# Deltares/pyflwdir

Measured on AMD Instinct MI355X. Metric: Mcells/s upstream_area on D8 raster, higher is better.
Workload: dtype int32

## Files before the change

pyflwdir_amd/csrc/tile_fast.h:

```cpp
#pragma once
#include <type_traits>

#define FX_SLOT0 (2u * TCELLS)
#define FX_NOBODY (FX_SLOT0 + 2u * PSL)
#define FX_PN (TCELLS + PSL + 8)
#ifndef FXP
#define FXP 4
#endif
#define FY_SINK0 (4u * TCELLS)

#define FX_TP_LO 0x3F404101u
#define FX_TP_HI 0xC1C0BFFFu
#define FX_TC_LO 0x47484901u
#define FX_TC_HI 0xB9B8B7FFu
#define FX_T0_LO 0xF7F70000u
#define FX_T0_HI 0xF7F7F7F7u

__device__ __forceinline__ u32 fx_ffbl(u32 x) {
  u32 r;
  asm("v_ffbl_b32 %0, %1" : "=v"(r) : "v"(x));
  return r;
}
__device__ __forceinline__ int fx_sext8(u32 x) { return (int)(int8_t)(x & 0xFFu); }

__device__ __forceinline__ u32 fx_rowmask(u32 lr) { return (lr == 0u ? 0xE0u : 0u) | (lr == TS - 1u ? 0x0Eu : 0u); }
__device__ __forceinline__ u32 fx_colmask(u32 lc) { return (lc == 0u ? 0x38u : 0u) | (lc == TS - 1u ? 0x83u : 0u); }

__device__ __forceinline__ bool fx_vote(u32 (*s_flag)[4], int round, u32 tid, bool live) {
  const bool any = __ballot(live) != 0ull;
  if ((tid & 63u) == 0u) s_flag[round & 1][tid >> 6] = any ? 1u : 0u;
  __syncthreads();
  const uint4 f = *(const uint4 *)s_flag[round & 1];
  return (f.x | f.y | f.z | f.w) != 0u;
}

struct NbrTab {
  uint16_t v[PSL][8];
};
constexpr NbrTab make_nbr_tab() {
  NbrTab t{};
  for (int p = 0; p < PSL; ++p) {
    int lr = 0, lc = 0;
    if (p < TS) lr = 0, lc = p;
    else if (p < 2 * TS) lr = TS - 1, lc = p - TS;
    else if (p < 2 * TS + (TS - 2)) lr = p - 2 * TS + 1, lc = 0;
    else lr = p - (2 * TS + (TS - 2)) + 1, lc = TS - 1;
    int cnt = 0;
    for (int k = 0; k < 8 && p < NPERIM; ++k) {
      const int dr = (k >= 1 && k <= 3) ? 1 : (k >= 5 ? -1 : 0);
      const int dc = (k == 0 || k == 1 || k == 7) ? 1 : ((k >= 3 && k <= 5) ? -1 : 0);
      const int nr = lr + dr, nc = lc + dc;
      if (nr >= 0 && nr < TS && nc >= 0 && nc < TS) continue;
      const int qr = nr & (TS - 1), qc = nc & (TS - 1);
      const int ps = qr == 0 ? qc : (qr == TS - 1 ? TS + qc : (qc == 0 ? 2 * TS + (qr - 1) : 2 * TS + (TS - 2) + (qr - 1)));
      const int d = 3 * ((nr < 0 ? -1 : (nr >= TS ? 1 : 0)) + 1) + (nc < 0 ? -1 : (nc >= TS ? 1 : 0)) + 1;
      t.v[p][cnt++] = (uint16_t)(ps | (d << 8) | (k << 12));
    }
    for (; cnt < 8; ++cnt) t.v[p][cnt] = (uint16_t)((p < NPERIM ? p : 0) | (4 << 8) | (8 << 12));
  }
  return t;
}
static __device__ __constant__ const NbrTab NBR_TAB = make_nbr_tab();

__device__ __forceinline__ u64 w_cell(u64 base, u32 f, u32 c) { return base + (u64)(__umulhi(c + 1u, f) - __umulhi(c, f)); }


template <int NW>
__device__ __forceinline__ bool fx_vote_n(u32 (*s_flag)[8], int round, u32 tid, bool live) {
  const bool any = __ballot(live) != 0ull;
  if ((tid & 63u) == 0u) s_flag[round & 1][tid >> 6] = any ? 1u : 0u;
  __syncthreads();
  const uint4 f = *(const uint4 *)s_flag[round & 1];
  u32 acc = f.x | f.y | f.z | f.w;
  if (NW == 8) {
    const uint4 g = *(const uint4 *)&s_flag[round & 1][4];
    acc |= g.x | g.y | g.z | g.w;
  }
  return acc != 0u;
}

template <bool RAW, bool WEIGHTS, bool WIDE = false>
__global__ void __launch_bounds__(256) k_tile_local_fast(TileArgs a) {
  __shared__ __attribute__((aligned(16))) u32 A[PSL * FXP];
  __shared__ __attribute__((aligned(16))) u64 A64[WIDE ? PSL * 4 : 2];
  __shared__ __attribute__((aligned(16))) uint16_t P[FX_PN];
  __shared__ __attribute__((aligned(16))) u8 code[HW * CP];
  __shared__ __attribute__((aligned(16))) u32 s_flag[2][4];
  __shared__ u64 s_cnt[4];
  const u32 tid = threadIdx.x;
  u32 bx_, by_;
  pfd_tile_of_block(&bx_, &by_);
  const u32 tc = bx_ + a.tc_lo, tr = by_ + a.tr_lo;
  const u32 sbase = sslot_base(tr, tc, a.nstc);
  const i64 r0 = (i64)tr * TS, c0 = (i64)tc * TS;
  bool mvq = false;
  {
    u32 v[5];
    stage_load_interior(RAW ? a.raw : a.ncode, a.ncol, r0, c0, tid, v);
    if (RAW) {
#pragma unroll
      for (int k = 0; k < 5; ++k) {
        const u32 x = v[k] ^ 0xF7F7F7F7u;
        mvq |= ((x - 0x01010101u) & ~x & 0x80808080u) != 0u;
      }
    }
    stage_store(code, tid, v);
  }
  *(uint4 *)&A[FXP * tid] = make_uint4(0u, 0u, 0u, 0u);
  if (FXP == 8) *(uint4 *)&A[FXP * tid + 4] = make_uint4(0u, 0u, 0u, 0u);
  if (WIDE) {
#pragma unroll
    for (int k = 0; k < 4; ++k) A64[tid + 256u * k] = 0;
  }
  P[TCELLS + tid] = (uint16_t)(FX_SLOT0 + 2u * tid);
  if (tid == 0) P[TCELLS + PSL] = (uint16_t)FX_NOBODY;
  const bool tile_mv = RAW ? (__syncthreads_or(mvq ? 1 : 0) != 0) : (__syncthreads(), false);

  const u32 qs = (tid >> 3) & 3u;
  const u32 lcq = 4u * (tid & 15u);
  u32 sh[4], cm[4];
#pragma unroll
  for (int s = 0; s < 4; ++s) {
    const u32 b = (u32)s ^ qs;
    sh[s] = 8u * b;
    cm[s] = fx_colmask(lcq + b);
  }
  u32 ndir = 0, npit = 0, nbad = 0;
  auto decode = [&](auto chk) {
  constexpr bool CHKMV = decltype(chk)::value;
#pragma unroll
  for (int j = 0; j < QPT; ++j) {
    const u32 lr = (tid >> 4) + 16u * j;
    const u32 l0 = 4u * tid + 1024u * j;
    const u32 ca0 = (lr + 1u) * CP + lcq + 4u;
    const u32 c4 = *(const u32 *)&code[ca0];
    const u32 rm = (j == 0 || j == QPT - 1) ? fx_rowmask(lr) : 0u;
    u32 p[4], n4 = 0, badq = 0;
#pragma unroll
    for (int s = 0; s < 4; ++s) {
      const u32 c = (c4 >> sh[s]) & 0xFFu;
      const u32 k = fx_ffbl(c);
      const u32 pcnt = __popc(c);
      bool isdir = pcnt == 1u;
      if (RAW) {
        if (CHKMV) {
          const u32 t = code[(u32)((int)(ca0 + (sh[s] >> 3)) + fx_sext8(__builtin_amdgcn_perm(FX_TC_HI, FX_TC_LO, k)))];
          isdir = isdir && t != D8_MV;
        }
        const u32 t0 = __builtin_amdgcn_perm(FX_T0_HI, FX_T0_LO, pcnt);
        const u32 n = isdir ? c : t0;
        badq |= t0 & ~c;
        n4 |= n << sh[s];
        ndir += isdir ? 1u : 0u;
        npit += n == 0u ? 1u : 0u;
      }
      const bool go = isdir && (c & (rm | cm[s])) == 0u;
      const u32 lt = (u32)((int)(l0 + (sh[s] >> 3)) + fx_sext8(__builtin_amdgcn_perm(FX_TP_HI, FX_TP_LO, k)));
      p[s] = go ? (PHYS(lt) << 1) : FX_NOBODY;
    }
    *(uint2 *)&P[l0] = make_uint2(p[0] | (p[1] << 16), p[2] | (p[3] << 16));
    if (RAW) {
      if (badq) {
#pragma unroll
        for (int s = 0; s < 4; ++s) {
          const u32 c = (c4 >> sh[s]) & 0xFFu;
          nbad += (__builtin_amdgcn_perm(FX_T0_HI, FX_T0_LO, __popc(c)) & ~c) ? 1u : 0u;
        }
      }
      *(u32 *)&code[ca0] = n4;
      __builtin_memcpy(a.ncode_w + (size_t)(r0 + lr) * a.ncol + (size_t)(c0 + lcq), &n4, 4);
    }
  }
  };
  if (RAW && tile_mv) decode(std::true_type{});
  else decode(std::false_type{});
  if (RAW) {
    u64 pk = (u64)(ndir + npit) | ((u64)npit << 16) | ((u64)nbad << 32);
    for (int o = 32; o > 0; o >>= 1) pk += __shfl_down(pk, o);
    if ((tid & 63u) == 0) s_cnt[tid >> 6] = pk;
  }
  __syncthreads();
  if (RAW && tid == 0) a.tcnt[(size_t)tr * a.ntc + tc] = s_cnt[0] + s_cnt[1] + s_cnt[2] + s_cnt[3];

  u32 xt12 = XR_NONE;
  int plr = 0, plc = 0;
  if (tid < NPERIM) {
    pslot_inv((int)tid, &plr, &plc);
    const u32 c = CODE(plr, plc);
    if (d8_is_dir(c)) {
      const int k = d8_slot(c);
      const int nr = plr + d8_dr(k), nc = plc + d8_dc(k);
      if ((unsigned)nr >= TS || (unsigned)nc >= TS) {
        xt12 = xr_t12(nr, nc);
        P[PHYS((u32)(plr * TS + plc))] = (uint16_t)(FX_SLOT0 + 2u * tid);
      }
    }
  }
  __syncthreads();

  u32 pc[QPT * 4];
  bool lv[QPT];
#pragma unroll
  for (int j = 0; j < QPT; ++j) {
    const uint2 pp = *(const uint2 *)&P[4u * tid + 1024u * j];
    pc[4 * j + 0] = pp.x & 0xFFFFu;
    pc[4 * j + 1] = pp.x >> 16;
    pc[4 * j + 2] = pp.y & 0xFFFFu;
    pc[4 * j + 3] = pp.y >> 16;
    lv[j] = !(pp.x & pp.y & (pp.x >> 16) & (pp.y >> 16) & FX_SLOT0);
  }
  int round = 0;
#pragma nounroll
  for (; round < MAXROUNDS_TILE; ++round) {
#pragma unroll
    for (int j = 0; j < QPT; ++j) {
      if (lv[j]) {
        u32 q[4];
#pragma unroll
        for (int b = 0; b < 4; ++b) q[b] = *(const uint16_t *)((const u8 *)P + pc[4 * j + b]);
#pragma unroll
        for (int b = 0; b < 4; ++b) q[b] = *(const uint16_t *)((const u8 *)P + q[b]);
#pragma unroll
        for (int b = 0; b < 4; ++b) pc[4 * j + b] = q[b];
        lv[j] = !(q[0] & q[1] & q[2] & q[3] & FX_SLOT0);
        *(uint2 *)&P[4u * tid + 1024u * j] = make_uint2(q[0] | (q[1] << 16), q[2] | (q[3] << 16));
      }
    }
    if (!fx_vote(s_flag, round, tid, lv[0] | lv[1] | lv[2] | lv[3])) break;
  }
  const u32 live = (lv[0] ? 1u : 0u) + (lv[1] ? 1u : 0u) + (lv[2] ? 1u : 0u) + (lv[3] ? 1u : 0u);
  if ((a.flags & 32) && tid == 0) {
    const unsigned long long r = (unsigned long long)min(round + 1, MAXROUNDS_TILE);
    const u32 w = (tr * a.ntc + tc) & 255u;
    atomicMax((unsigned long long *)&a.rcnt[w], r);
    atomicAdd((unsigned long long *)&a.rcnt[256 + w], r);
  }
  if (live) atomicAdd((unsigned long long *)&a.ctrl[T_UNSAT], (unsigned long long)live);

  const u32 rep = 4u * (tid & (FXP - 1u));
#pragma unroll
  for (int j = 0; j < QPT; ++j) {
    u32 x[4], w[4];
#pragma unroll
    for (int s = 0; s < 4; ++s) {
      x[s] = pc[4 * j + s] - FX_SLOT0;
      w[s] = x[s] < 2u * PSL ? 1u : 0u;
      if (WEIGHTS) {
        const u32 lr = (tid >> 4) + 16u * j;
        w[s] = x[s] < 2u * PSL ? (u32)a.weights[(size_t)(r0 + lr) * a.ncol + (size_t)(c0 + lcq + (sh[s] >> 3))] : 0u;
      }
    }
    const bool e10 = x[1] == x[0], e20 = x[2] == x[0], e21 = x[2] == x[1], e30 = x[3] == x[0], e31 = x[3] == x[1], e32 = x[3] == x[2];
    w[0] += (e10 ? w[1] : 0u) + (e20 ? w[2] : 0u) + (e30 ? w[3] : 0u);
    w[1] = e10 ? 0u : w[1] + ((!e20 && e21) ? w[2] : 0u) + ((!e30 && e31) ? w[3] : 0u);
    w[2] = (e20 || e21) ? 0u : w[2] + ((!e30 && !e31 && e32) ? w[3] : 0u);
    w[3] = (e30 || e31 || e32) ? 0u : w[3];
#pragma unroll
    for (int s = 0; s < 4; ++s)
      if (w[s]) atomicAdd((u32 *)((u8 *)A + (x[s] << (FXP == 8 ? 4 : 3)) + rep), w[s]);
    if (WIDE) {
      const u32 lr = (tid >> 4) + 16u * j;
      const u64 wr = a.wrow[(u32)(r0 + lr)];
      const u32 wf = a.wfrac[(u32)(r0 + lr)];
      u64 v[4];
#pragma unroll
      for (int s = 0; s < 4; ++s) v[s] = x[s] < 2u * PSL ? w_cell(wr, wf, (u32)c0 + lcq + (sh[s] >> 3)) : 0ull;
      const bool e10 = x[1] == x[0], e20 = x[2] == x[0], e21 = x[2] == x[1], e30 = x[3] == x[0], e31 = x[3] == x[1], e32 = x[3] == x[2];
      v[0] += (e10 ? v[1] : 0ull) + (e20 ? v[2] : 0ull) + (e30 ? v[3] : 0ull);
      v[1] = e10 ? 0ull : v[1] + ((!e20 && e21) ? v[2] : 0ull) + ((!e30 && e31) ? v[3] : 0ull);
      v[2] = (e20 || e21) ? 0ull : v[2] + ((!e30 && !e31 && e32) ? v[3] : 0ull);
      v[3] = (e30 || e31 || e32) ? 0ull : v[3];
#pragma unroll
      for (int s = 0; s < 4; ++s)
        if (v[s]) atomicAdd((unsigned long long *)&A64[(x[s] >> 1) * 4u + (tid & 3u)], (unsigned long long)v[s]);
    }
  }
  __syncthreads();

  u32 xt = 0, link = XR_NONE, inmask = 0;
  if (tid < NPERIM) {
    if (xt12 != XR_NONE) {
      const uint4 lo = *(const uint4 *)&A[tid * FXP];
      xt = lo.x + lo.y + lo.z + lo.w;
      if (FXP == 8) {
        const uint4 hi = *(const uint4 *)&A[tid * FXP + 4];
        xt += hi.x + hi.y + hi.z + hi.w;
      }
    }
    const u32 c = CODE(plr, plc);
    if (c != D8_MV) {
#pragma unroll
      for (int k = 0; k < 8; ++k) {
        const int nr = plr + d8_dr(k), nc = plc + d8_dc(k);
        if (((unsigned)nr >= TS || (unsigned)nc >= TS) && CODE(nr, nc) == (1u << ((k + 4) & 7))) inmask |= 1u << k;
      }
    }
    if (inmask) {
      const u32 x = (u32)P[PHYS((u32)(plr * TS + plc))] - FX_SLOT0;
      if (x < 2u * PSL) link = x >> 1;
    }
  }
  a.xT[sbase + tid] = xt;
  a.xrec[sbase + tid] = xr_pack(xt12 & 0xFFu, xt12 >> 8, link, inmask);
  if (WIDE) a.xT64[sbase + tid] = (tid < NPERIM && xt12 != XR_NONE) ? A64[4u * tid] + A64[4u * tid + 1] + A64[4u * tid + 2] + A64[4u * tid + 3] : 0ull;
  const u64 xm = __ballot(xt12 != XR_NONE);
  if ((tid & 63u) == 0u) a.xmask[(sbase + tid) >> 6] = xm;
}

template <bool WEIGHTS, int NT>
__global__ void __launch_bounds__(NT, NT == 256 ? 6 : 8) k_tile_final_fast(TileArgs a) {
  constexpr int QF = TCELLS / 4 / NT;
  constexpr u32 QSTR = 4u * NT;
  constexpr u32 RSTR = NT / 16;
  constexpr int NW = NT / 64;
  __shared__ __attribute__((aligned(16))) u32 A[TCELLS + 64];
  __shared__ __attribute__((aligned(16))) uint16_t P[TCELLS + 64];
  __shared__ __attribute__((aligned(16))) u32 s_flag[2][8];
  const u32 tid = threadIdx.x;
  u32 bx_, by_;
  pfd_tile_of_block(&bx_, &by_);
  const u32 tc = bx_ + a.tc_lo, tr = by_ + a.tr_lo;
  const u32 sbase = sslot_base(tr, tc, a.nstc);
  const i64 r0 = (i64)tr * TS, c0 = (i64)tc * TS;
  const u32 lcq = 4u * (tid & 15u);
  u32 cq[QF];
#pragma unroll
  for (int j = 0; j < QF; ++j)
    __builtin_memcpy(&cq[j], a.ncode + (size_t)(r0 + (tid >> 4) + RSTR * j) * a.ncol + (size_t)(c0 + lcq), 4);
  const u32 ptid = tid & 255u;
  const u32 rec = tid < 256u ? a.xrec[sbase + ptid] : 0u;
  u32 xc[5], xk[5];
  {
    const uint4 nb = *reinterpret_cast<const uint4 *>(NBR_TAB.v[ptid]);
    const u32 dl = min(tid & 15u, 8u), ql = (dl * 11u) >> 5;
    const u32 nbase = sslot_base(tr + ql - 1u, tc + (dl - 3u * ql) - 1u, a.nstc);
    const u32 e5[5] = {nb.x & 0xFFFFu, nb.x >> 16, nb.y & 0xFFFFu, nb.y >> 16, nb.z & 0xFFFFu};
#pragma unroll
    for (int i = 0; i < 5; ++i) {
      const u32 bs = (u32)__shfl((int)nbase, (int)(((tid & 48u) | ((e5[i] >> 8) & 15u))));
      xc[i] = a.xtot[bs + (e5[i] & 0xFFu)];
      xk[i] = e5[i] >> 12;
    }
  }
  const u32 sink = FY_SINK0 + 4u * (tid & 63u);
  if (tid < 64u) P[TCELLS + tid] = (uint16_t)sink;

  const u32 qs = (tid >> 3) & 3u;
  u32 sh[4], cm[4];
#pragma unroll
  for (int s = 0; s < 4; ++s) {
    const u32 b = (u32)s ^ qs;
    sh[s] = 8u * b;
    cm[s] = fx_colmask(lcq + b);
  }
  u32 pc[QF * 4], qn[QF * 4];
  bool lv[QF];
#pragma unroll
  for (int j = 0; j < QF; ++j) {
    const u32 lr = (tid >> 4) + RSTR * j;
    const u32 l0 = 4u * tid + QSTR * j;
    const u32 c4 = cq[j];
    const u32 rm = (j == 0 || j == QF - 1) ? fx_rowmask(lr) : 0u;
    u32 w4[4];
#pragma unroll
    for (int s = 0; s < 4; ++s) {
      const u32 c = (c4 >> sh[s]) & 0xFFu;
      const bool go = __popc(c & ~(rm | cm[s])) == 1u;
      const u32 lt = (u32)((int)(l0 + (sh[s] >> 3)) + fx_sext8(__builtin_amdgcn_perm(FX_TP_HI, FX_TP_LO, fx_ffbl(c))));
      pc[4 * j + s] = go ? (PHYS(lt) << 2) : sink;
      u32 wv = 1u;
      if (WEIGHTS) wv = (u32)a.weights[(size_t)(r0 + lr) * a.ncol + (size_t)(c0 + lcq + (sh[s] >> 3))];
      w4[s] = c != D8_MV ? wv : 0u;
    }
    *(uint4 *)&A[l0] = make_uint4(w4[0], w4[1], w4[2], w4[3]);
    *(uint2 *)&P[l0] = make_uint2(pc[4 * j + 0] | (pc[4 * j + 1] << 16), pc[4 * j + 2] | (pc[4 * j + 3] << 16));
    lv[j] = !(pc[4 * j + 0] & pc[4 * j + 1] & pc[4 * j + 2] & pc[4 * j + 3] & FY_SINK0);
  }
  u32 inf = 0;
  {
    const u32 m = (rec >> 16) & 0xFFu;
#pragma unroll
    for (int i = 0; i < 5; ++i) inf += ((m >> xk[i]) & 1u) ? xc[i] : 0u;
  }
  __syncthreads();
  if (inf) {
    int plr, plc;
    pslot_inv((int)ptid, &plr, &plc);
    A[PHYS((u32)(plr * TS + plc))] += inf;
  }
  __syncthreads();

#define FY_ROUND(PC, QN)                                                                                                \
  {                                                                                                               \
    u32 av[QF * 4];                                                                                              \
    _Pragma("unroll") for (int j = 0; j < QF; ++j) {                                                              \
      if (lv[j]) {                                                                                                \
        const uint4 a4 = *(const uint4 *)&A[4u * tid + QSTR * j];                                                  \
        av[4 * j + 0] = a4.x, av[4 * j + 1] = a4.y, av[4 * j + 2] = a4.z, av[4 * j + 3] = a4.w;                   \
        _Pragma("unroll") for (int b = 0; b < 4; ++b)                                                             \
            QN[4 * j + b] = *(const uint16_t *)((const u8 *)P + (PC[4 * j + b] >> 1));                           \
      }                                                                                                           \
    }                                                                                                             \
    __syncthreads();                            \
    _Pragma("unroll") for (int j = 0; j < QF; ++j) {                                                              \
      if (lv[j]) {                                                                                                \
         \
         \
        const u32 t0 = PC[4 * j], t1 = PC[4 * j + 1], t2 = PC[4 * j + 2], t3 = PC[4 * j + 3];                     \
        u32 w0 = av[4 * j], w1 = av[4 * j + 1], w2 = av[4 * j + 2], w3 = av[4 * j + 3];                           \
        const bool e10 = t1 == t0, e20 = t2 == t0, e21 = t2 == t1, e30 = t3 == t0, e31 = t3 == t1, e32 = t3 == t2; \
        w0 += (e10 ? w1 : 0u) + (e20 ? w2 : 0u) + (e30 ? w3 : 0u);                                                \
        w1 = e10 ? 0u : w1 + ((!e20 && e21) ? w2 : 0u) + ((!e30 && e31) ? w3 : 0u);                               \
        w2 = (e20 || e21) ? 0u : w2 + ((!e30 && !e31 && e32) ? w3 : 0u);                                          \
        w3 = (e30 || e31 || e32) ? 0u : w3;                                                                       \
        atomicAdd((u32 *)((u8 *)A + t0), w0);                                                                     \
        if (w1) atomicAdd((u32 *)((u8 *)A + t1), w1);                                                             \
        if (w2) atomicAdd((u32 *)((u8 *)A + t2), w2);                                                             \
        if (w3) atomicAdd((u32 *)((u8 *)A + t3), w3);                                                             \
        lv[j] = !(QN[4 * j + 0] & QN[4 * j + 1] & QN[4 * j + 2] & QN[4 * j + 3] & FY_SINK0);                      \
        *(uint2 *)&P[4u * tid + QSTR * j] =                                                                       \
            make_uint2(QN[4 * j + 0] | (QN[4 * j + 1] << 16), QN[4 * j + 2] | (QN[4 * j + 3] << 16));             \
      }                                                                                                           \
    }                                                                                                             \
  }
  auto anylive = [&]() {
    bool v = false;
    _Pragma("unroll") for (int j = 0; j < QF; ++j) v |= lv[j];
    return v;
  };
  int round = 0;
#pragma nounroll
  for (; round < MAXROUNDS_TILE; round += 2) {
    FY_ROUND(pc, qn)
    if (!fx_vote_n<NW>(s_flag, 0, tid, anylive())) break;
    FY_ROUND(qn, pc)
    if (!fx_vote_n<NW>(s_flag, 1, tid, anylive())) {
      ++round;
      break;
    }
  }
#undef FY_ROUND
  u32 live = 0;
  _Pragma("unroll") for (int j = 0; j < QF; ++j) live += lv[j] ? 1u : 0u;
  if ((a.flags & 32) && tid == 0) {
    const unsigned long long r = (unsigned long long)min(round + 1, MAXROUNDS_TILE);
    const u32 w = (tr * a.ntc + tc) & 255u;
    atomicMax((unsigned long long *)&a.rcnt[512 + w], r);
    atomicAdd((unsigned long long *)&a.rcnt[768 + w], r);
  }
  if (live) atomicAdd((unsigned long long *)&a.ctrl[T_UNSAT], (unsigned long long)live);

#pragma unroll
  for (int j = 0; j < QF; ++j) {
    const u32 l0 = 4u * tid + QSTR * j;
    const u32 c4 = cq[j];
    const uint4 a4 = *(const uint4 *)&A[l0];
    const u32 x0 = (qs & 1u) ? a4.y : a4.x, x1 = (qs & 1u) ? a4.x : a4.y;
    const u32 x2 = (qs & 1u) ? a4.w : a4.z, x3 = (qs & 1u) ? a4.z : a4.w;
    i32 o4[4] = {(i32)((qs & 2u) ? x2 : x0), (i32)((qs & 2u) ? x3 : x1), (i32)((qs & 2u) ? x0 : x2),
                 (i32)((qs & 2u) ? x1 : x3)};
#pragma unroll
    for (int b = 0; b < 4; ++b)
      if (((c4 >> (8 * b)) & 0xFFu) == D8_MV) o4[b] = -9999;
    i32 *dst = a.out + (size_t)(r0 + (tid >> 4) + RSTR * j - a.row_first) * a.ncol + (size_t)(c0 + lcq);
    if ((((size_t)dst) & 15) == 0) {
      *(int4 *)dst = make_int4(o4[0], o4[1], o4[2], o4[3]);
    } else {
#pragma unroll
      for (int b = 0; b < 4; ++b) dst[b] = o4[b];
    }
  }
}
```

Baseline: 214,800.

## Use ds_write_addtid stores and split even/odd planes for tile pointer array

```diff
diff --git a/pyflwdir_amd/csrc/tile_fast.h b/pyflwdir_amd/csrc/tile_fast.h
--- a/pyflwdir_amd/csrc/tile_fast.h
+++ b/pyflwdir_amd/csrc/tile_fast.h
@@ -79,6 +79,25 @@
   return acc != 0u;
 }
 
+__device__ __forceinline__ u32 fx_lds_addr(const void *p) {
+  return (u32)(__UINTPTR_TYPE__)(__attribute__((address_space(3))) const void *)p;
+}
+#pragma clang diagnostic push
+#pragma clang diagnostic ignored "-Winline-asm"
+__device__ __forceinline__ void fx_st_addtid(u32 m0, u32 d) {
+  asm volatile("s_mov_b32 m0, %1\n\ts_nop 0\n\tds_write_addtid_b32 %0" : : "v"(d), "s"(m0) : "m0", "memory");
+}
+__device__ __forceinline__ void fx_st2_addtid(u32 m0, u32 d0, u32 d1) {
+  asm volatile("s_mov_b32 m0, %2\n\ts_nop 0\n\tds_write_addtid_b32 %0\n\tds_write_addtid_b32 %1 offset:4096"
+               :
+               : "v"(d0), "v"(d1), "s"(m0)
+               : "m0", "memory");
+}
+#pragma clang diagnostic pop
+__device__ __forceinline__ void fx_lds_drain() { asm volatile("s_waitcnt lgkmcnt(0)" : : : "memory"); }
+
+#define FX_PB(z) ((z) + 4095u * ((z) & 1u))
+
 template <bool RAW, bool WEIGHTS, bool WIDE = false>
 __global__ void __launch_bounds__(256) k_tile_local_fast(TileArgs a) {
   __shared__ __attribute__((aligned(16))) u32 A[PSL * FXP];
@@ -93,6 +112,7 @@
   const u32 tc = bx_ + a.tc_lo, tr = by_ + a.tr_lo;
   const u32 sbase = sslot_base(tr, tc, a.nstc);
   const i64 r0 = (i64)tr * TS, c0 = (i64)tc * TS;
+  const u32 wv256 = 256u * (u32)__builtin_amdgcn_readfirstlane((int)(tid >> 6));
   bool mvq = false;
   {
     u32 v[5];
@@ -104,27 +124,26 @@
         mvq |= ((x - 0x01010101u) & ~x & 0x80808080u) != 0u;
       }
     }
-    stage_store(code, tid, v);
-  }
-  *(uint4 *)&A[FXP * tid] = make_uint4(0u, 0u, 0u, 0u);
-  if (FXP == 8) *(uint4 *)&A[FXP * tid + 4] = make_uint4(0u, 0u, 0u, 0u);
+#pragma unroll
+    for (int k = 0; k < 5; ++k)
+      if (tid + 256u * k < HW * 18u) fx_st_addtid(fx_lds_addr(code) + wv256 + 1024u * k, v[k]);
+  }
+#pragma unroll
+  for (int k = 0; k < FXP; ++k) fx_st_addtid(fx_lds_addr(A) + wv256 + 1024u * k, 0u);
   if (WIDE) {
 #pragma unroll
-    for (int k = 0; k < 4; ++k) A64[tid + 256u * k] = 0;
-  }
-  P[TCELLS + tid] = (uint16_t)(FX_SLOT0 + 2u * tid);
-  if (tid == 0) P[TCELLS + PSL] = (uint16_t)FX_NOBODY;
+    for (int k = 0; k < 8; ++k) fx_st_addtid(fx_lds_addr(A64) + wv256 + 1024u * k, 0u);
+  }
+  if (tid <= PSL / 2u) {
+    const u32 w0 = FX_SLOT0 + 4u * tid;
+    fx_st_addtid(fx_lds_addr(P) + FX_SLOT0 + wv256, w0 | ((w0 + 2u) << 16));
+  }
+  fx_lds_drain();
   const bool tile_mv = RAW ? (__syncthreads_or(mvq ? 1 : 0) != 0) : (__syncthreads(), false);
 
-  const u32 qs = (tid >> 3) & 3u;
   const u32 lcq = 4u * (tid & 15u);
-  u32 sh[4], cm[4];
-#pragma unroll
-  for (int s = 0; s < 4; ++s) {
-    const u32 b = (u32)s ^ qs;
-    sh[s] = 8u * b;
-    cm[s] = fx_colmask(lcq + b);
-  }
+  const u32 sh[4] = {0u, 8u, 16u, 24u};
+  const u32 cm[4] = {lcq == 0u ? 0x38u : 0u, 0u, 0u, lcq == TS - 4u ? 0x83u : 0u};
   u32 ndir = 0, npit = 0, nbad = 0;
   auto decode = [&](auto chk) {
   constexpr bool CHKMV = decltype(chk)::value;
@@ -156,9 +175,9 @@
       }
       const bool go = isdir && (c & (rm | cm[s])) == 0u;
       const u32 lt = (u32)((int)(l0 + (sh[s] >> 3)) + fx_sext8(__builtin_amdgcn_perm(FX_TP_HI, FX_TP_LO, k)));
-      p[s] = go ? (PHYS(lt) << 1) : FX_NOBODY;
-    }
-    *(uint2 *)&P[l0] = make_uint2(p[0] | (p[1] << 16), p[2] | (p[3] << 16));
+      p[s] = go ? FX_PB(lt) : FX_NOBODY;
+    }
+    fx_st2_addtid(fx_lds_addr(P) + wv256 + 1024u * j, p[0] | (p[2] << 16), p[1] | (p[3] << 16));
     if (RAW) {
       if (badq) {
 #pragma unroll
@@ -167,7 +186,7 @@
           nbad += (__builtin_amdgcn_perm(FX_T0_HI, FX_T0_LO, __popc(c)) & ~c) ? 1u : 0u;
         }
       }
-      *(u32 *)&code[ca0] = n4;
+      if (n4 != c4) *(u32 *)&code[ca0] = n4;
       __builtin_memcpy(a.ncode_w + (size_t)(r0 + lr) * a.ncol + (size_t)(c0 + lcq), &n4, 4);
     }
   }
@@ -179,6 +198,7 @@
     for (int o = 32; o > 0; o >>= 1) pk += __shfl_down(pk, o);
     if ((tid & 63u) == 0) s_cnt[tid >> 6] = pk;
   }
+  fx_lds_drain();
   __syncthreads();
   if (RAW && tid == 0) a.tcnt[(size_t)tr * a.ntc + tc] = s_cnt[0] + s_cnt[1] + s_cnt[2] + s_cnt[3];
 
@@ -192,7 +212,7 @@
       const int nr = plr + d8_dr(k), nc = plc + d8_dc(k);
       if ((unsigned)nr >= TS || (unsigned)nc >= TS) {
         xt12 = xr_t12(nr, nc);
-        P[PHYS((u32)(plr * TS + plc))] = (uint16_t)(FX_SLOT0 + 2u * tid);
+        *(uint16_t *)((u8 *)P + FX_PB((u32)(plr * TS + plc))) = (uint16_t)(FX_SLOT0 + 2u * tid);
       }
     }
   }
@@ -202,10 +222,10 @@
   bool lv[QPT];
 #pragma unroll
   for (int j = 0; j < QPT; ++j) {
-    const uint2 pp = *(const uint2 *)&P[4u * tid + 1024u * j];
+    const uint2 pp = make_uint2(((const u32 *)P)[tid + 256u * j], ((const u32 *)P)[TCELLS / 4 + tid + 256u * j]);
     pc[4 * j + 0] = pp.x & 0xFFFFu;
-    pc[4 * j + 1] = pp.x >> 16;
-    pc[4 * j + 2] = pp.y & 0xFFFFu;
+    pc[4 * j + 2] = pp.x >> 16;
+    pc[4 * j + 1] = pp.y & 0xFFFFu;
     pc[4 * j + 3] = pp.y >> 16;
     lv[j] = !(pp.x & pp.y & (pp.x >> 16) & (pp.y >> 16) & FX_SLOT0);
   }
@@ -223,9 +243,10 @@
 #pragma unroll
         for (int b = 0; b < 4; ++b) pc[4 * j + b] = q[b];
         lv[j] = !(q[0] & q[1] & q[2] & q[3] & FX_SLOT0);
-        *(uint2 *)&P[4u * tid + 1024u * j] = make_uint2(q[0] | (q[1] << 16), q[2] | (q[3] << 16));
-      }
-    }
+        fx_st2_addtid(fx_lds_addr(P) + wv256 + 1024u * j, q[0] | (q[2] << 16), q[1] | (q[3] << 16));
+      }
+    }
+    fx_lds_drain();
     if (!fx_vote(s_flag, round, tid, lv[0] | lv[1] | lv[2] | lv[3])) break;
   }
   const u32 live = (lv[0] ? 1u : 0u) + (lv[1] ? 1u : 0u) + (lv[2] ? 1u : 0u) + (lv[3] ? 1u : 0u);
@@ -296,7 +317,7 @@
       }
     }
     if (inmask) {
-      const u32 x = (u32)P[PHYS((u32)(plr * TS + plc))] - FX_SLOT0;
+      const u32 x = (u32) * (const uint16_t *)((const u8 *)P + FX_PB((u32)(plr * TS + plc))) - FX_SLOT0;
       if (x < 2u * PSL) link = x >> 1;
     }
   }
```

Result: no change. 216,700 (median of 6 runs) (+0.9%).
